# ilirlikalla/Smith-Waterman-FPGA-module

Hardware: AMD Instinct MI355X
Metric: GCUPS (higher is better)
Workload: dtype f16

## Files before the change

### smith-waterman-fpga-module_amd/csrc/swbank_bank.h

```cpp
#ifndef SWBANK_BANK_H
#define SWBANK_BANK_H

#include <dlfcn.h>
#include <hip/hip_runtime.h>
#include <rccl/rccl.h>

#include <algorithm>
#include <cmath>
#include <cstdarg>
#include <cstdio>
#include <cstdlib>
#include <cstring>
#include <atomic>
#include <condition_variable>
#include <functional>
#include <memory>
#include <mutex>
#include <numeric>
#include <thread>
#include <chrono>
#include <vector>
#if defined(__SSE2__)
#include <emmintrin.h>
#endif
// ... 219 lines not shown
      if (stop_.load()) return;
      (*job_)(i);
      pending_.fetch_sub(1, std::memory_order_acq_rel);
    }
  }
  unsigned n_;
  std::vector<std::thread> th_;
  std::mutex m_;
  std::condition_variable cv_;
  const std::function<void(unsigned)>* job_ = nullptr;
  std::atomic<unsigned> pending_{0};
  std::atomic<uint64_t> gen_{0};
  std::atomic<bool> stop_{false};
};

class Launcher {
 public:
  explicit Launcher(int device) : th_([this, device] { loop(device); }) {}
  ~Launcher() {
    {
      std::lock_guard<std::mutex> g(m_);
      stop_ = true;
    }
    cv_.notify_one();
    th_.join();
  }
  void post(std::function<sw_status()> f) {
    {
      std::lock_guard<std::mutex> g(m_);
      q_.push_back(std::move(f));
      ++posted_;
    }
    cv_.notify_one();
  }
  sw_status wait(size_t k) {
    while (done_.load(std::memory_order_acquire) < k) {
#if defined(__SSE2__)
      _mm_pause();
#endif
    }
    return st_.load(std::memory_order_acquire);
  }
  sw_status wait_all() { return wait(posted_); }
  void reset() {
    wait_all();
    posted_ = 0;
    done_.store(0);
    st_.store(SW_OK);
  }

 private:
  void loop(int device) {
    (void)hipSetDevice(device);
    for (;;) {
      std::function<sw_status()> f;
      {
        std::unique_lock<std::mutex> l(m_);
        cv_.wait(l, [&] { return stop_ || !q_.empty(); });
        if (q_.empty()) return;
        f = std::move(q_.front());
        q_.erase(q_.begin());
      }
      if (st_.load(std::memory_order_relaxed) == SW_OK) {
        const sw_status s = f();
        if (s != SW_OK) st_.store(s, std::memory_order_release);
      }
      done_.fetch_add(1, std::memory_order_acq_rel);
    }
  }
  std::mutex m_;
  std::condition_variable cv_;
  std::vector<std::function<sw_status()>> q_;
  bool stop_ = false;
  size_t posted_ = 0;
  std::atomic<size_t> done_{0};
  std::atomic<sw_status> st_{SW_OK};
  std::thread th_;
};

struct sw_bank {
  sw_config cfg{};
  int device = 0;
  int cus = 0;
  hipStream_t stream = nullptr;
  char err[512] = {0};

  bool have_pen = false;
  int alpha = SW_DNA_ALPHA;
  std::vector<int8_t> matrix;
  int32_t gap_open = 0, gap_extend = 0;

  bool have_query = false;
  uint64_t qid = 0;
  std::vector<uint8_t> query;
  std::vector<std::vector<uint8_t>> qset;
  bool mq_ready = false;
  DevBuf<uint32_t> mqtab, mqtab16;
  size_t mq_words = 0;
  DevBuf<uint32_t> mqpair;
  size_t mq_pair_words = 0;
  int mq_pair_segs = 0, mq_pair_rows = 0;
  uint32_t mq_pS1 = 0, mq_pS2 = 0;

  bool dirty = true;
  int R = 32, RB = 4, W = 1, col0 = 0, prof = 0;
  uint32_t S = 0, O = 0, E = 0, nv = 0, PS = 0, pad = 4;
  int32_t smax = 0;
  DevBuf<uint32_t> qtab;
  bool f16 = false;
  uint32_t nv16 = 0, PS16 = 0;
  int32_t f16_neg = 0;
  DevBuf<uint32_t> qtab16;
  DevBuf<uint32_t> qpair;
  uint32_t pair_bytes = 0, pS1 = 0, pS2 = 0;
  DevBuf<uint32_t> fb_idx, fb_cnt;
  bool i32_ready = false;
  uint32_t i32_strips = 0;
  DevBuf<uint2> i32prof, i32scr;
  DevBuf<unsigned long long> best_key;
  struct Seg { int W; size_t off, off16; };
  std::vector<Seg> segs;
  DevBuf<uint2> edge[2];
  int wK = 0;
  int wsegs = 1;
  size_t wseg_words = 0, wseg_words16 = 0;
  uint32_t wPS = 0;
  DevBuf<uint32_t> wtab;
  DevBuf<uint32_t> wtab16;
  uint32_t wPS16 = 0;
  int sK[3] = {0, 0, 0};
  size_t sseg_words[3] = {0, 0, 0}, sseg_words16[3] = {0, 0, 0};
  uint32_t sPS[3] = {0, 0, 0}, sPS16[3] = {0, 0, 0};
  DevBuf<uint32_t> stab[3], stab16[3];
  DevBuf<uint2> sring;
  DevBuf<uint32_t> tprog;

  static constexpr int NSLOT = 3, NDSLOT = 6;
  hipStream_t copy_stream = nullptr;
  hipEvent_t h2d_done[NSLOT] = {}, kern_done[NDSLOT] = {};
  PinBuf hslot[NSLOT], hscores;
  std::vector<std::vector<uint32_t>> mlist;
  std::vector<std::vector<uint8_t>> mstage;
  std::vector<std::vector<uint32_t>> mbad;
  std::vector<hipEvent_t> out_ev;
  hipStream_t out_stream = nullptr;
  hipStream_t stream2 = nullptr;
  hipEvent_t ev_s2 = nullptr;
  double host_pack_ms = 0;
  int feed_dslots = NSLOT;
  DevBuf<uint8_t> dslot[NDSLOT];
  DevBuf<uint32_t> sortscr[NDSLOT];
  DevBuf<uint8_t> sbuf;
  UcBuf sflag;
  DevBuf<SwkStreamChunk> sdrec;
  DevBuf<uint32_t> sctr;
  hipStream_t kstream = nullptr;
  PinBuf srec, shflag{hipHostMallocCoherent};
  PinBuf shscores{hipHostMallocCoherent};
  std::vector<hipEvent_t> sev;
  std::unique_ptr<HostPool> pool;
  std::unique_ptr<Launcher> launcher;

  DevBuf<uint8_t> res;
  DevBuf<uint64_t> offs;
  DevBuf<uint32_t> lens;
  DevBuf<int32_t> scores;
  DevBuf<uint8_t> gres;
  DevBuf<uint64_t> goffs;
  DevBuf<uint32_t> glens;

  char last_kernel[160] = {0};

  int best_kind = 0;
  uint64_t best_id = 0, best_index = 0;
  int32_t best_score = 0;
  DevBuf<uint64_t> best_dev;
  hipEvent_t best_ev = nullptr;

  std::vector<sw_bank*> kids;
  std::unique_ptr<HostPool> dpool;
  std::vector<void*> comms;
  bool rccl_gather = false;
  unsigned pool_threads = 0;
  DevBuf<int32_t> grecv;
  PinBuf hrecv;
  DevBuf<uint32_t> bal_state, bal_flag;
  DevBuf<uint32_t> wbal_state, wbal_flag;
  uint32_t wbal_gen = 0;
  DevBuf<uint32_t> bal_plan;
  size_t bal_key[3] = {0, 0, 0};
  uint32_t bal_gen = 0;
  bool peer_ready = false;
  hipEvent_t ev_join = nullptr;
  std::vector<hipEvent_t> deal_ev;
  bool best_root = false;
  DevBuf<uint32_t> dperm, dsort;
  bool is_multi() const { return !kids.empty(); }
  bool gotoh() const { return cfg.gap_model == SW_GAP_GOTOH; }

  hipEvent_t ev_ready = nullptr, ev_used = nullptr;
  PinBuf stage;

  sw_counters ctr{};

  PinBuf faultw{hipHostMallocCoherent};
  bool host_call = false;
  bool no_handoff = false;

  bool timing = false;
  struct Ev { hipEvent_t a, b, c; };
  std::vector<Ev> events;
};

struct DevGuard {
  int prev = -1;
  DevGuard() {
    if (hipGetDevice(&prev) != hipSuccess) prev = -1;
  }
  explicit DevGuard(const sw_bank* b) : DevGuard() {
    if (b && b->device >= 0) (void)hipSetDevice(b->device);
  }
  ~DevGuard() {
    if (prev >= 0) (void)hipSetDevice(prev);
  }
  DevGuard(const DevGuard&) = delete;
  DevGuard& operator=(const DevGuard&) = delete;
};

inline uint16_t f16_score_bits(int v) {
  return __builtin_bit_cast(uint16_t, (_Float16)((float)v * (1.0f / 2048.0f)));
}


sw_status fail(sw_bank* b, sw_status st, const char* fmt, ...);

#define HIPOK(bank, expr)                                                                 \
  do {                                                                                    \
    hipError_t e_ = (expr);                                                               \
    if (e_ != hipSuccess)                                                                 \
      return fail((bank), SW_ERR_HIP, "%s: %s (%s:%d)", #expr, hipGetErrorString(e_),    \
                  __FILE__, __LINE__);                                                    \
  } while (0)

struct Rccl {
  bool ok = false;
  char err[160] = {0};
  decltype(&ncclCommInitAll) commInitAll = nullptr;
  decltype(&ncclCommDestroy) commDestroy = nullptr;
  decltype(&ncclGather) gather = nullptr;
  decltype(&ncclGetErrorString) errorString = nullptr;
  decltype(&ncclCommAbort) commAbort = nullptr;
  decltype(&ncclCommGetAsyncError) asyncError = nullptr;
  decltype(&ncclGroupStart) groupStart = nullptr;
  decltype(&ncclGroupEnd) groupEnd = nullptr;
};
const Rccl& rccl();

template <class F>
sw_status each_kid(sw_bank* b, F&& f) {
  for (sw_bank* k : b->kids) {
    const sw_status st = f(k);
    if (st != SW_OK) return fail(b, st, "device %d: %s", k->device, k->err);
  }
  return SW_OK;
}

unsigned host_threads();

template <class F>
void parallel_for(HostPool& pool, size_t n, F&& f) {
  const unsigned T = pool.size();
  if (T <= 1 || n < 2048) {
    f((size_t)0, n);
    return;
  }
  const size_t step = (n + T - 1) / T;
  pool.run([&](unsigned p) {
    const size_t lo = std::min(n, p * step), hi = std::min(n, lo + step);
    if (lo < hi) f(lo, hi);
  });
}

inline size_t align16(size_t x) { return (x + 15) & ~(size_t)15; }
inline uint32_t record_len(const uint8_t* rec) {
  uint16_t l;
  std::memcpy(&l, rec + 4, 2);
  return l;
}

void copy_kernel_name(sw_bank* b, const char* gather);
uint32_t* fault_word(sw_bank* b);
sw_status take_fault(sw_bank* b, int which);
sw_status prepare(sw_bank* b);
sw_status prepare_multi(sw_bank* b);
sw_status prepare_i32(sw_bank* b);
void u16_gotoh_rows(const sw_bank* b, bool f16, int& R, int& W);
bool wave_preferred(const sw_bank* b, size_t n, uint32_t max_len, bool use_f16);
sw_status launch(sw_bank* b, const uint8_t* d_res, const uint64_t* d_offs,
                 const uint32_t* d_lens, size_t n, uint32_t max_len, int32_t* d_scores,
                 hipStream_t st, uint32_t packed = SWK_PACK_BYTES,
                 const uint32_t* perm = nullptr, const uint32_t* perm_n = nullptr,
                 bool dsort = false, bool wait_prev = true, uint32_t* sort_out = nullptr,
                 uint32_t* sort_scr = nullptr, uint32_t ulen = 0, uint32_t ustride = 0,
                 uint32_t min_len = 0);
bool chunk_perm(HostPool& pool, const uint32_t* len, size_t n, uint32_t* perm);
bool scratch_free(const sw_bank* b, uint32_t max_len);
struct MixedOrder {
  std::vector<uint32_t> pos;
  uint32_t hi = 0, shift = 0, nbin = 0;
};
bool mixed_pack(sw_bank* b, const uint8_t* residues, size_t nres, const uint64_t* offsets,
                const uint32_t* lens, size_t c0, size_t cnt, size_t step,
// ... 25 lines not shown
```

### smith-waterman-fpga-module_amd/csrc/swbank_bank.hip

```cpp
#include "swbank_bank.h"

sw_status fail(sw_bank* b, sw_status st, const char* fmt, ...) {
  if (b) {
    va_list ap;
    va_start(ap, fmt);
    vsnprintf(b->err, sizeof(b->err), fmt, ap);
    va_end(ap);
  }
  return st;
}

extern "C" int32_t sw_device_count(void) {
  int n = 0;
  if (hipGetDeviceCount(&n) != hipSuccess) return 0;
  return n;
}

static sw_status check_device(int dev) {
  int ndev = 0;
  if (hipGetDeviceCount(&ndev) != hipSuccess || ndev <= 0) return SW_ERR_NO_DEVICE;
  if (dev < 0 || dev >= ndev) return SW_ERR_NO_DEVICE;
  hipDeviceProp_t prop;
  if (hipGetDeviceProperties(&prop, dev) != hipSuccess) return SW_ERR_NO_DEVICE;
  if (std::strncmp(prop.gcnArchName, "gfx950", 6) != 0) return SW_ERR_NO_DEVICE;
// ... 37 lines not shown
      }
      k->pool_threads = std::max(2u, host_threads() / (unsigned)cfg.n_devices);
      b->kids.push_back(k);
    }
    b->dpool.reset(new (std::nothrow) HostPool((unsigned)cfg.n_devices));
    b->pool.reset(new (std::nothrow) HostPool(host_threads()));
    if (!b->dpool || !b->pool) {
      sw_bank_destroy(b);
      return SW_ERR_NOMEM;
    }
    const char* gm = std::getenv("SWBANK_GATHER");
    const bool force_copy = gm && std::strcmp(gm, "copy") == 0;
    const bool force_rccl = gm && std::strcmp(gm, "rccl") == 0;
    bool distinct = true;
    for (int i = 0; i < cfg.n_devices; ++i)
      for (int j = 0; j < i; ++j) distinct = distinct && cfg.devices[i] != cfg.devices[j];
    if (!force_copy && (distinct || force_rccl)) {
      const Rccl& r = rccl();
      ncclResult_t nr = ncclSuccess;
      if (r.ok) {
        std::vector<ncclComm_t> comms((size_t)cfg.n_devices);
        nr = r.commInitAll(comms.data(), cfg.n_devices, cfg.devices);
        if (nr == ncclSuccess) b->comms.assign(comms.begin(), comms.end());
      }
      b->rccl_gather = !b->comms.empty();
      if (b->comms.empty() && force_rccl) {
        sw_bank_destroy(b);
        return SW_ERR_UNSUPPORTED;
      }
      if (b->comms.empty())
        snprintf(b->err, sizeof(b->err), "RCCL unavailable (%s), gathering with device copies",
                 r.ok ? r.errorString(nr) : r.err);
    }
    (void)hipSetDevice(b->device);
    *out = b;
    return SW_OK;
  }

  int dev = cfg.device;
  if (dev < 0 && hipGetDevice(&dev) != hipSuccess) return SW_ERR_NO_DEVICE;
  const sw_status dst = check_device(dev);
  if (dst != SW_OK) return dst;

  sw_bank* b = new (std::nothrow) sw_bank();
  if (!b) return SW_ERR_NOMEM;
  b->cfg = cfg;
  b->device = dev;
  if (hipSetDevice(dev) != hipSuccess ||
      hipStreamCreateWithFlags(&b->stream, hipStreamNonBlocking) != hipSuccess ||
      hipStreamCreateWithFlags(&b->copy_stream, hipStreamNonBlocking) != hipSuccess ||
      hipStreamCreateWithFlags(&b->out_stream, hipStreamNonBlocking) != hipSuccess ||
      hipStreamCreateWithFlags(&b->stream2, hipStreamNonBlocking) != hipSuccess) {
    for (hipStream_t* x : {&b->stream, &b->copy_stream, &b->out_stream, &b->stream2})
      if (*x) (void)hipStreamDestroy(*x);
    delete b;
    return SW_ERR_HIP;
  }
  b->alpha = cfg.alphabet == SW_ALPHABET_DNA ? SW_DNA_ALPHA : SW_PROTEIN_ALPHA;
  if (hipDeviceGetAttribute(&b->cus, hipDeviceAttributeMultiprocessorCount, dev) != hipSuccess)
    b->cus = 0;
  if (cfg.alphabet == SW_ALPHABET_PROTEIN) {
    int8_t m[SW_PROTEIN_ALPHA * SW_PROTEIN_ALPHA];
    sw_fill_matrix(SW_ALPHABET_PROTEIN, 0, 0, m);
    b->matrix.assign(m, m + sizeof(m));
    b->gap_open = -11;
    b->gap_extend = -1;
    b->have_pen = true;
  }
  *out = b;
  return SW_OK;
}

extern "C" void sw_bank_destroy(sw_bank* b) {
  DevGuard dev_guard(b);
  if (!b) return;
  if (b->is_multi() || !b->comms.empty()) {
    const Rccl& r = rccl();
    for (void* c : b->comms) (void)r.commDestroy(static_cast<ncclComm_t>(c));
    (void)hipSetDevice(b->device);
    if (b->ev_used) (void)hipEventSynchronize(b->ev_used);
    if (b->ev_join) (void)hipEventDestroy(b->ev_join);
    if (b->ev_used) (void)hipEventDestroy(b->ev_used);
    for (sw_bank* k : b->kids) sw_bank_destroy(k);
    b->dpool.reset();
    b->pool.reset();
    (void)hipSetDevice(b->device);
    b->grecv.release();
    b->hrecv.release();
    b->res.release();
    b->offs.release();
    b->lens.release();
    b->dperm.release();
    b->dsort.release();
    delete b;
    return;
  }
  (void)hipSetDevice(b->device);
  if (b->stream) (void)hipStreamSynchronize(b->stream);
  uint64_t nl;
  double pm, sm;
  (void)sw_bank_timing(b, &nl, &pm, &sm);
  b->faultw.release();
  b->qtab.release();
  b->qtab16.release();
  b->mqtab.release();
  b->mqtab16.release();
  b->mqpair.release();
  b->qpair.release();
  b->stage.release();
  if (b->ev_ready) (void)hipEventDestroy(b->ev_ready);
  if (b->ev_used) (void)hipEventDestroy(b->ev_used);
  if (b->best_ev) (void)hipEventDestroy(b->best_ev);
  if (b->ev_join) (void)hipEventDestroy(b->ev_join);
  for (hipEvent_t e : b->deal_ev) (void)hipEventDestroy(e);
  b->fb_idx.release();
  b->fb_cnt.release();
  b->best_key.release();
  b->best_dev.release();
  b->i32prof.release();
  b->i32scr.release();
  b->dperm.release();
  b->dsort.release();
  b->bal_state.release();
  b->bal_flag.release();
  b->wbal_state.release();
  b->wbal_flag.release();
  b->bal_plan.release();
  b->wtab.release();
  b->wtab16.release();
  b->tprog.release();
  for (int i = 0; i < 3; ++i) {
    b->stab[i].release();
    b->stab16[i].release();
  }
  b->sring.release();
  b->edge[0].release();
  b->edge[1].release();
  if (b->copy_stream) (void)hipStreamSynchronize(b->copy_stream);
  if (b->out_stream) (void)hipStreamSynchronize(b->out_stream);
  if (b->stream2) (void)hipStreamSynchronize(b->stream2);
  for (hipEvent_t e : b->out_ev) (void)hipEventDestroy(e);
  for (int i = 0; i < sw_bank::NSLOT; ++i) b->hslot[i].release();
  for (int i = 0; i < sw_bank::NDSLOT; ++i) {
    b->dslot[i].release();
    b->sortscr[i].release();
  }
  b->sbuf.release();
  b->sflag.release();
  b->sdrec.release();
  b->sctr.release();
  b->srec.release();
  b->shflag.release();
  b->shscores.release();
  for (hipEvent_t e : b->sev) (void)hipEventDestroy(e);
  for (int i = 0; i < sw_bank::NSLOT; ++i)
    if (b->h2d_done[i]) (void)hipEventDestroy(b->h2d_done[i]);
  for (int i = 0; i < sw_bank::NDSLOT; ++i)
    if (b->kern_done[i]) (void)hipEventDestroy(b->kern_done[i]);
  b->hscores.release();
  b->launcher.reset();
  b->pool.reset();
  if (b->copy_stream) (void)hipStreamDestroy(b->copy_stream);
  if (b->out_stream) (void)hipStreamDestroy(b->out_stream);
  if (b->stream2) (void)hipStreamDestroy(b->stream2);
  if (b->kstream) (void)hipStreamDestroy(b->kstream);
  if (b->ev_s2) (void)hipEventDestroy(b->ev_s2);
  b->res.release();
  b->offs.release();
  b->lens.release();
  b->scores.release();
  b->gres.release();
  b->goffs.release();
  b->glens.release();
  if (b->stream) (void)hipStreamDestroy(b->stream);
  delete b;
}

extern "C" int32_t sw_bank_devices(const sw_bank* b, int32_t* devices, int32_t cap) {
  if (!b) return 0;
  const int32_t n = b->is_multi() ? (int32_t)b->kids.size() : 1;
  for (int32_t i = 0; devices && i < std::min(n, cap); ++i)
    devices[i] = b->is_multi() ? b->kids[(size_t)i]->device : b->device;
  return n;
}

extern "C" const char* sw_last_error(const sw_bank* b) { return b ? b->err : "null bank"; }

extern "C" const char* sw_last_kernel(const sw_bank* b) { return b ? b->last_kernel : ""; }

uint32_t* fault_word(sw_bank* b) {
  if (!b->faultw.p) {
    if (b->faultw.reserve(64) != hipSuccess) return nullptr;
    std::memset(b->faultw.p, 0, b->faultw.cap);
  }
  return reinterpret_cast<uint32_t*>(b->faultw.p);
}

sw_status take_fault(sw_bank* b, int which) {
  if (b->is_multi()) {
    sw_status st = SW_OK;
    for (sw_bank* k : b->kids) {
      const sw_status ks = take_fault(k, which);
      if (ks != SW_OK && st == SW_OK) st = fail(b, ks, "device %d: %s", k->device, k->err);
    }
    return st;
  }
  if (!b->faultw.p) return SW_OK;
  volatile uint32_t* w = reinterpret_cast<volatile uint32_t*>(b->faultw.p) + which * SWK_FAULT_WORDS;
  uint32_t f = 0;
  for (int i = 0; i < SWK_FAULT_WORDS; ++i) {
    f |= w[i];
    w[i] = 0;
  }
  if (f == 0) return SW_OK;
  if (f & SWK_FAULT_BAL) ++b->ctr.balanced_timeouts;
  if (f & SWK_FAULT_TAIL) ++b->ctr.tail_timeouts;
  if (f & SWK_FAULT_WBAL) ++b->ctr.wave_balanced_timeouts;
  char kinds[96] = "";
  const char* names[3] = {"balanced ranges", "protein tail", "wave balanced ranges"};
  for (int i = 0; i < 3; ++i)
    if (f & (1u << i)) {
      if (kinds[0]) strncat(kinds, ", ", sizeof(kinds) - strlen(kinds) - 1);
      strncat(kinds, names[i], sizeof(kinds) - strlen(kinds) - 1);
    }
  return fail(b, SW_ERR_TIMEOUT,
              "a cross-workgroup hand-off wait ran out (%s) in a %s call: its scores are invalid",
              kinds, which ? "host-buffer" : "device");
}

extern "C" sw_status sw_bank_sync(sw_bank* b) {
  DevGuard dev_guard(b);
  if (!b) return SW_ERR_ARG;
  if (b->is_multi()) {
    for (sw_bank* k : b->kids) {
      const sw_status st = sw_bank_sync(k);
      if (st != SW_OK) {
        (void)take_fault(b, 0);
        return fail(b, st, "device %d: %s", k->device, k->err);
      }
    }
    if (b->ev_used) {
      int cur = -1;
      HIPOK(b, hipGetDevice(&cur));
      hipError_t e = hipSetDevice(b->device);
      if (e == hipSuccess) e = hipEventSynchronize(b->ev_used);
      (void)hipSetDevice(cur);
      HIPOK(b, e);
    }
    return SW_OK;
  }
  int cur = -1;
  HIPOK(b, hipGetDevice(&cur));
  hipError_t e = hipSetDevice(b->device);
  if (e == hipSuccess && b->ev_used) e = hipEventSynchronize(b->ev_used);
  if (e == hipSuccess) e = hipStreamSynchronize(b->stream);
  (void)hipSetDevice(cur);
  HIPOK(b, e);
  return take_fault(b, 0);
}

static void sum_counters(sw_counters& c, const sw_bank* b) {
  c.stream_calls += b->ctr.stream_calls;
  c.stream_reruns += b->ctr.stream_reruns;
  c.stream_declined += b->ctr.stream_declined;
  c.chunked_calls += b->ctr.chunked_calls;
  c.device_sorts += b->ctr.device_sorts;
  c.gather_timeouts += b->ctr.gather_timeouts;
  c.mixed_chunks += b->ctr.mixed_chunks;
  c.mixed_runs += b->ctr.mixed_runs;
  c.balanced_calls += b->ctr.balanced_calls;
  c.balanced_timeouts += b->ctr.balanced_timeouts;
  c.tail_timeouts += b->ctr.tail_timeouts;
  c.handoff_reruns += b->ctr.handoff_reruns;
  c.wave_balanced_timeouts += b->ctr.wave_balanced_timeouts;
  c.h2d_bytes += __atomic_load_n(&b->ctr.h2d_bytes, __ATOMIC_RELAXED);
}

extern "C" sw_status sw_bank_counters_ex(const sw_bank* b, sw_counters* out, size_t out_size) {
  if (!b || !out) return SW_ERR_ARG;
  if (out_size != 64 && out_size != 80 && out_size != 96 && out_size != sizeof(sw_counters))
    return SW_ERR_ARG;
  sw_counters c{};
  sum_counters(c, b);
  for (const sw_bank* k : b->kids) sum_counters(c, k);
  std::memcpy(out, &c, out_size);
  return SW_OK;
}

extern "C" sw_status sw_bank_counters(const sw_bank* b, sw_counters* out) {
  return sw_bank_counters_ex(b, out, 64);
}

void copy_kernel_name(sw_bank* b, const char* gather) {
  snprintf(b->last_kernel, sizeof(b->last_kernel), "multi[%zu] gather=%s: %s", b->kids.size(),
           gather, b->kids[0]->last_kernel);
}

static sw_status set_matrix_impl(sw_bank* b, const int8_t* m, int alpha, int32_t go,
                                 int32_t ge) {
  if (go > 0 || ge > 0 || go < -32767 || ge < -32767)
    return fail(b, SW_ERR_ARG, "gap penalties must be <= 0 (got open %d, extend %d)", go, ge);
  b->matrix.assign(m, m + (size_t)alpha * alpha);
  b->alpha = alpha;
  b->gap_open = go;
  b->gap_extend = ge;
  b->have_pen = true;
  b->dirty = true;
// ... 578 lines not shown
```

### smith-waterman-fpga-module_amd/csrc/swbank_kcommon.h

```cpp
#ifndef SWBANK_KCOMMON_H
#define SWBANK_KCOMMON_H
#include <hip/hip_runtime.h>
#include <stdint.h>

#include <algorithm>
#include <cstdlib>
#include <mutex>
#include <type_traits>
#include <vector>

#include "swbank_internal.h"

#ifndef SWK_TAIL_TOP
#define SWK_TAIL_TOP 1
#endif
#ifndef SWK_PRIO_ROT
#define SWK_PRIO_ROT 1
#endif
#ifndef SWK_PRIO_SHIFT
#define SWK_PRIO_SHIFT 18
#endif

#ifndef SWK_PRIO_END
#define SWK_PRIO_END 3
// ... 467 lines not shown
                                              uint32_t ulen, uint32_t ustride) {
  Lane2 t;
  size_t a = (size_t)tile * SWB_TILE + lane, b = a + 64;
  const bool va = a < n, vb = b < n;
  const size_t p0 = (size_t)tile * SWB_TILE;
  if (p0 >= n) {
    t.llo = t.lhi = 0u;
    t.plo = t.phi = packed == SWK_PACK_RECORDS || ustride ? res + (packed ? 6 : 0)
                                                          : reinterpret_cast<const uint8_t*>(lens);
    return t;
  }
  if (!va) a = p0;
  if (!vb) b = p0;
  if (idx) {
    a = idx[a];
    b = idx[b];
  }
  if (packed == SWK_PACK_RECORDS) {
    t.llo = va ? record_len(res + a * SWB_RECORD) : 0u;
    t.lhi = vb ? record_len(res + b * SWB_RECORD) : 0u;
    t.plo = res + a * SWB_RECORD + 6;
    t.phi = res + b * SWB_RECORD + 6;
    return t;
  }
  if (ustride) {
    t.llo = va ? ulen : 0u;
    t.lhi = vb ? ulen : 0u;
    t.plo = res + a * ustride;
    t.phi = res + b * ustride;
    return t;
  }
  const uint32_t la = lens[a], lb = lens[b];
  t.llo = va ? la : 0u;
  t.lhi = vb ? lb : 0u;
  if constexpr (MIX) {
    if (packed == SWK_PACK_MIXED) {
      const uint32_t* o32 = reinterpret_cast<const uint32_t*>(offs);
      t.plo = la ? mixed_ptr(res, o32[a]) : reinterpret_cast<const uint8_t*>(lens);
      t.phi = lb ? mixed_ptr(res, o32[b]) : reinterpret_cast<const uint8_t*>(lens);
      return t;
    }
  }
  t.plo = la ? res + offs[a] : reinterpret_cast<const uint8_t*>(lens);
  t.phi = lb ? res + offs[b] : reinterpret_cast<const uint8_t*>(lens);
  return t;
}

template <int C = 8>
__device__ __forceinline__ void tile_chunks(const Lane2& t, size_t tlo, size_t thi, size_t n,
                                            int& nch, int& nfull, int& ncl) {
  uint32_t Lmax = max(t.llo, t.lhi);
  uint32_t Lmin = min(tlo < n ? t.llo : ~0u, thi < n ? t.lhi : ~0u);
#pragma unroll
  for (int off = 32; off >= 1; off >>= 1) {
    Lmax = max(Lmax, (uint32_t)__shfl_xor((int)Lmax, off));
    Lmin = min(Lmin, (uint32_t)__shfl_xor((int)Lmin, off));
  }
  const int lx = (int)__builtin_amdgcn_readfirstlane(Lmax);
  nch = max(1, (lx + C - 1) / C);
  ncl = lx == 0 ? C : lx - C * (nch - 1);
  const uint32_t lm = __builtin_amdgcn_readfirstlane(Lmin);
  nfull = lm == ~0u ? 0 : (int)(lm / C);
}

struct ScoreArgs {
  const uint8_t* res;
  const uint64_t* offs;
  const uint32_t* lens;
  size_t n;
  const uint32_t* qtab;
  uint32_t nv;
  uint32_t S, O, E;
  uint32_t PS;
  uint32_t pad;
  int32_t* scores;
  const uint2* edge_in;
  uint2* edge_out;
  uint32_t ecols;
  uint32_t accum;
  uint32_t packed;
  const uint32_t* idx;
  const uint32_t* nidx;
  uint32_t idx_base;
  const uint32_t* ident;
  uint32_t pS1, pS2;
  uint32_t f16_noe, f16_ne, f16_no;
  const uint32_t* fb_qtab;
  uint32_t fb_nv, fb_PS;
  int32_t fb_thresh;
  uint32_t split_blocks;
  uint32_t split_P;
  uint32_t main_pairs;
  const uint32_t* split_qtab;
  const uint32_t* split_fb_qtab;
  uint32_t split_words, split_fb_words, split_PS, split_fb_PS;
  uint2* split_ring;
  uint32_t ulen, ustride;
  uint32_t nq, qwords;
  size_t sstride;
  const SwkStreamChunk* sc;
  const uint32_t* hflag;
  uint32_t* dflag;
  uint32_t* tctr;
  uint32_t nsc;
  uint32_t* bal_flag;
  uint32_t* bal_state;
  const uint4* bal_plan;
  uint32_t bal_gen;
  uint32_t* tail_prog;
  uint32_t tail_pairs, tail_cols;
  uint32_t* fault;
  uint32_t poll_limit, stall;
  uint32_t wbal_blocks, wbal_grid;
  const uint32_t* sidx;
};
static_assert(sizeof(ScoreArgs) == 376, "ScoreArgs layout (kernel argument block) changed");

__device__ __forceinline__ void report_fault(uint32_t* fault, uint32_t bit) {
  if (fault) __hip_atomic_store(fault + __builtin_ctz(bit), bit, __ATOMIC_RELAXED,
                                __HIP_MEMORY_SCOPE_SYSTEM);
}

typedef __attribute__((address_space(3))) void* lds_void_ptr;
typedef __attribute__((address_space(1))) void* glob_void_ptr;

template <int C = 8>
__device__ __forceinline__ void dma_edge_chunk(const uint2* src, uint2* dst, int lane) {
#pragma unroll
  for (int q = 0; q < C / 2; ++q)
    __builtin_amdgcn_global_load_lds((glob_void_ptr)(src + q * 128 + lane * 2),
                                     (lds_void_ptr)(dst + q * 128), 16, 0, 0);
}

template <int C = 8>
__device__ __forceinline__ int tile_nch(const uint8_t* res, const uint32_t* lens, size_t n,
                                        int tile, int lane, uint32_t packed, const uint32_t* idx,
                                        uint32_t ulen, uint32_t ustride) {
  const size_t a = (size_t)tile * SWB_TILE + lane, b = a + 64;
  auto len = [&](size_t k) -> uint32_t {
    if (k >= n) return 0u;
    if (ustride) return ulen;
    if (idx) k = idx[k];
    return packed == SWK_PACK_RECORDS ? record_len(res + k * SWB_RECORD) : lens[k];
  };
  uint32_t L = max(len(a), len(b));
#pragma unroll
  for (int off = 32; off >= 1; off >>= 1) L = max(L, (uint32_t)__shfl_xor((int)L, off));
  return max(1, (int)((__builtin_amdgcn_readfirstlane(L) + C - 1) / C));
}

#ifndef SWK_STREAM_POLL
#define SWK_STREAM_POLL 64
#endif
#ifndef SWK_STREAM_POLL_ALL
#define SWK_STREAM_POLL_ALL 0
#endif
__device__ __forceinline__ uint32_t stream_mode(const uint32_t* hflag, uint32_t* dflag, int c,
                                                int nsc, int lane) {
  for (int it = 0; it < (1 << 20); ++it) {
    uint32_t v = __builtin_amdgcn_readfirstlane(
        __hip_atomic_load(dflag + c, __ATOMIC_ACQUIRE, __HIP_MEMORY_SCOPE_AGENT));
    if (v) {
      __builtin_amdgcn_fence(__ATOMIC_ACQUIRE, "");
      return v;
    }
    if ((SWK_STREAM_POLL_ALL || threadIdx.x < 64) &&
        (it == 0 || ((it + (int)blockIdx.x) % SWK_STREAM_POLL) == 0)) {
      v = __builtin_amdgcn_readfirstlane(
          __hip_atomic_load(hflag + c, __ATOMIC_ACQUIRE, __HIP_MEMORY_SCOPE_SYSTEM));
      if (v) {
        if (lane == 0) __hip_atomic_store(dflag + c, v, __ATOMIC_RELEASE, __HIP_MEMORY_SCOPE_AGENT);
        return v;
      }
    }
    __builtin_amdgcn_s_sleep(16);
  }
  if (lane == 0) {
    __hip_atomic_store(dflag + c, SWK_STREAM_ABORT, __ATOMIC_RELAXED, __HIP_MEMORY_SCOPE_AGENT);
    __hip_atomic_store(const_cast<uint32_t*>(hflag) + nsc + c, SWK_STREAM_ABORT,
                       __ATOMIC_RELAXED, __HIP_MEMORY_SCOPE_SYSTEM);
  }
  return SWK_STREAM_ABORT;
}


inline int cached_occupancy(const void* fn, int threads, size_t lds, int dev, int* cus) {
  struct Entry { const void* fn; int threads; size_t lds; int dev, occ, cus; };
  static std::mutex m;
  static std::vector<Entry> cache;
  std::lock_guard<std::mutex> g(m);
  for (const Entry& e : cache)
    if (e.fn == fn && e.threads == threads && e.lds == lds && e.dev == dev) {
      *cus = e.cus;
      return e.occ;
    }
  int occ = 0, c = 0;
  if (hipDeviceGetAttribute(&c, hipDeviceAttributeMultiprocessorCount, dev) != hipSuccess ||
      hipOccupancyMaxActiveBlocksPerMultiprocessor(&occ, fn, threads, lds) != hipSuccess)
    return 0;
  cache.push_back({fn, threads, lds, dev, occ, c});
  *cus = c;
  return occ;
}

inline unsigned persistent_grid(const void* fn, size_t ntiles, int threads, size_t lds) {
  int dev = 0, cus = 0;
  if (hipGetDevice(&dev) != hipSuccess) return (unsigned)ntiles;
  const int occ = cached_occupancy(fn, threads, lds, dev, &cus);
  if (cus <= 0 || occ <= 0) return (unsigned)ntiles;
  const size_t slots = (size_t)cus * occ;
  const size_t rounds = (ntiles + slots - 1) / slots;
  return (unsigned)((ntiles + rounds - 1) / rounds);
}

}
#endif
```

### smith-waterman-fpga-module_amd/csrc/swbank_stream.hip

```cpp
#include "swbank_bank.h"

sw_status stream_feed(sw_bank* b, const uint8_t* residues, size_t nres,
                      const uint64_t* offsets, size_t n, uint32_t L, int32_t* out, bool& used,
                      const uint8_t* recs, const uint32_t* rlens) {
  used = false;
  if (recs && (L == 0 || L > SWB_RECORD_MAX)) return SW_OK;
  const int mode_env = env_int("SWBANK_STREAM", 1);
  if (mode_env == 0 || !out || b->alpha != SW_DNA_ALPHA || b->prof || b->col0 || b->RB != 4 ||
      env_int("SWBANK_PACK2", 1) == 0 || env_int("SWBANK_UNIFORM", 1) == 0 ||
      !scratch_free(b, L) || n > 0x7FFFFFFFull)
    return SW_OK;
  if (rlens && env_int("SWBANK_MIXED", 1) == 0) return SW_OK;
  const char* kforce = std::getenv("SWBANK_KERNEL");
  if (kforce && std::strcmp(kforce, "wave") == 0) return SW_OK;
  const size_t T = (n + SWB_TILE - 1) / SWB_TILE;
  if (mode_env != 2 && T < 8 * (size_t)std::max(b->cus, 1)) return SW_OK;
  const uint64_t smax = (uint64_t)std::max(0, b->smax);
  const bool use_f16 = b->f16 && b->f16_neg >= -2048 && env_int("SWBANK_F16", 1) != 0 &&
                       std::min<uint64_t>(b->query.size(), L) * smax + smax <= 2048u;
  const bool pair = use_f16 && b->pair_bytes != 0 && env_int("SWBANK_PAIR", 1) != 0;
  if (!(b->R == 16 || b->R == 32)) return SW_OK;
  int sR = b->R, sW = b->segs[0].W;
  u16_gotoh_rows(b, use_f16, sR, sW);

  std::vector<size_t> tile0;
  const size_t cap = std::max<size_t>(1, T / 8);
  for (size_t t = 0, sz = std::max<size_t>(1, T / 64); t < T; t += sz, sz = std::min(cap, 2 * sz))
    tile0.push_back(t);
  const size_t nsc = tile0.size();
  tile0.push_back(T);
  const size_t nib = (L + 1) / 2;
  const size_t PT0 = b->pool ? b->pool->size() : 1;
  std::vector<size_t> roff(nsc + 1, 0);
  size_t slot_bytes = 0, zbytes = 0;
  for (size_t i = 0; i < nsc; ++i) {
    const size_t cnt = std::min(n, tile0[i + 1] * SWB_TILE) - tile0[i] * SWB_TILE;
    const size_t head = rlens ? align16(cnt * 12) : 0;
    const size_t body = rlens ? cnt * ((L + 3) / 4) + cnt * (size_t)L / 32 + cnt * nib + 32 * PT0
                              : cnt * nib;
    if (rlens && head + body + 64 >= ((size_t)1 << 29)) return SW_OK;
    roff[i + 1] = roff[i] + (head + body + 64 + 255) / 256 * 256;
    slot_bytes = std::max(slot_bytes, roff[i + 1] - roff[i]);
    zbytes = std::max(zbytes, head + 64);
  }
  if (!rlens) zbytes = 0;
  const size_t cap_bytes = (size_t)std::max(1, env_int("SWBANK_STREAM_MB", 4096)) << 20;
  if (roff[nsc] + zbytes + n * 4 > cap_bytes) {
    ++b->ctr.stream_declined;
    return SW_OK;
  }
  HIPOK(b, hipSetDevice(b->device));
  if (!b->kstream) {
    if (b->cus <= 0) return SW_OK;
    std::vector<uint32_t> mask(((size_t)b->cus + 31) / 32, 0xFFFFFFFFu);
    if (hipExtStreamCreateWithCUMask(&b->kstream, (uint32_t)mask.size(), mask.data()) !=
        hipSuccess) {
      b->kstream = nullptr;
      (void)hipGetLastError();
      return SW_OK;
    }
  }
  hipStream_t ks = b->kstream;
  {
    bool ok = b->sbuf.reserve(roff[nsc] + zbytes) == hipSuccess &&
              b->sflag.reserve(nsc * 4) == hipSuccess &&
              b->sdrec.reserve(nsc) == hipSuccess && b->sctr.reserve(1) == hipSuccess &&
              b->srec.reserve(nsc * sizeof(SwkStreamChunk)) == hipSuccess &&
              b->shflag.reserve(nsc * 8) == hipSuccess &&
              b->shscores.reserve(n * 4) == hipSuccess;
    for (int i = 0; ok && i < std::min<int>(sw_bank::NSLOT, (int)nsc); ++i)
      ok = b->hslot[i].reserve(slot_bytes) == hipSuccess;
    while (ok && b->sev.size() < nsc) {
      hipEvent_t e;
      ok = hipEventCreateWithFlags(&e, hipEventDisableTiming | hipEventBlockingSync) == hipSuccess;
      if (ok) b->sev.push_back(e);
    }
    if (!ok) {
      (void)hipGetLastError();
      b->sbuf.release();
      b->shscores.release();
      ++b->ctr.stream_declined;
      return SW_OK;
    }
  }
  used = true;
  SwkStreamChunk* rec = reinterpret_cast<SwkStreamChunk*>(b->srec.p);
  uint32_t* hflag = reinterpret_cast<uint32_t*>(b->shflag.p);
  for (size_t i = 0; i < nsc; ++i) {
    rec[i] = SwkStreamChunk{(unsigned)tile0[i], (unsigned)roff[i], (unsigned)(roff[i] >> 32),
                            (unsigned)(roff[nsc] / 256)};
    __atomic_store_n(&hflag[i], 0u, __ATOMIC_RELAXED);
    __atomic_store_n(&hflag[nsc + i], 0u, __ATOMIC_RELAXED);
  }
  std::atomic_thread_fence(std::memory_order_seq_cst);

  sw_bank::Ev ev{};
  const auto start_kernel = [&]() -> sw_status {
    HIPOK(b, hipStreamWaitEvent(ks, b->ev_ready, 0));
    HIPOK(b, hipStreamWaitEvent(ks, b->ev_used, 0));
    HIPOK(b, hipMemcpyAsync(b->sdrec.p, rec, nsc * sizeof(SwkStreamChunk), hipMemcpyHostToDevice,
                            ks));
    HIPOK(b, hipMemsetAsync(b->sflag.p, 0, nsc * 4, ks));
    HIPOK(b, hipMemsetAsync(b->sctr.p, 0, 4, ks));
    if (zbytes) HIPOK(b, hipMemsetAsync(b->sbuf.p + roff[nsc], 0, zbytes, ks));
    if (b->timing) {
      HIPOK(b, hipEventCreate(&ev.a));
      HIPOK(b, hipEventCreate(&ev.c));
      HIPOK(b, hipEventRecord(ev.a, ks));
      ev.b = ev.a;
    }
    HIPOK(b, swk_launch_stream(sR, b->gotoh() ? 1 : 0, use_f16 ? 1 : 0, pair ? 1 : 0, b->sbuf.p,
                               n, rlens ? 0u : L, b->sdrec.p, hflag,
                               reinterpret_cast<uint32_t*>(b->sflag.p),
                               (uint32_t)nsc, b->sctr.p,
                               pair ? b->qpair.p : use_f16 ? b->qtab16.p : b->qtab.p,
                               use_f16 ? b->nv16 : b->nv, b->S, b->O, b->E,
                               pair ? b->pair_bytes : 0, b->pad, sW,
                               reinterpret_cast<int32_t*>(b->shscores.p),
                               b->pS1, b->pS2, ks));
    HIPOK(b, hipEventRecord(b->ev_used, ks));
    if (b->timing) {
      HIPOK(b, hipEventRecord(ev.c, ks));
      b->events.push_back(ev);
    }
    snprintf(b->last_kernel, sizeof(b->last_kernel), "tile %s%s R=%d W=%d segs=1 streamed=%zu",
             use_f16 ? "f16" : "u16", pair ? " pair" : "", sR, sW, nsc);
    trace_mark("kernel");
    return SW_OK;
  };

  std::vector<uint32_t> mode(nsc, 0);
  size_t issued = 0;
  bool stop = false;
  std::mutex pm;
  std::condition_variable pcv;
  const int hold_ms = env_int("SWBANK_STREAM_HOLD_MS", 0);
  std::vector<std::chrono::steady_clock::time_point> pub_t(nsc);
  size_t published = 0;
  hipError_t pub_err = hipSuccess;
  std::thread publisher([&] {
    for (size_t i = 0; i < nsc; ++i) {
      {
        std::unique_lock<std::mutex> lk(pm);
        pcv.wait(lk, [&] { return issued > i || stop; });
        if (issued <= i) return;
      }
      const hipError_t e = hipEventSynchronize(b->sev[i]);
      if (e != hipSuccess) {
        pub_err = e;
        for (size_t j = i; j < nsc; ++j) __atomic_store_n(&hflag[j], SWK_STREAM_ABORT, __ATOMIC_RELEASE);
        return;
      }
      if (i == 1 && hold_ms > 0) std::this_thread::sleep_for(std::chrono::milliseconds(hold_ms));
      __atomic_store_n(&hflag[i], mode[i], __ATOMIC_RELEASE);
      pub_t[i] = std::chrono::steady_clock::now();
      published = i + 1;
    }
  });

  HostPool& pool = *b->pool;
  const unsigned PT = pool.size();
  const bool avx2 = env_int("SWBANK_AVX2", 1) != 0;
  const swpack::PackFn pack2fn = swpack::packer(2, avx2), pack4fn = swpack::packer(4, avx2);
  const size_t steps32 = (L + 31u) / 32u;
  bool nib_mode = false;
  std::atomic<size_t> oob{SIZE_MAX};
  std::vector<uint64_t> rbase(PT), rspan(PT);
  std::vector<size_t> psz(PT + 1, 0), p4(PT + 1, 0);
  const bool runs_ok = env_int("SWBANK_MIXED_RUNS", 1) != 0;
  MixedOrder mo;
  if (rlens) {
    mo.hi = L;
    while ((L >> mo.shift) >= 1024u) ++mo.shift;
    mo.nbin = (L >> mo.shift) + 1;
    mo.pos.assign((size_t)PT * mo.nbin, 0u);
  }
  std::atomic<uint32_t> wide{0};
  sw_status err = SW_OK;
  bool started = false;
  bool nonuniform = false;
  for (size_t i = 0; i < nsc && err == SW_OK; ++i) {
    const int s = (int)(i % sw_bank::NSLOT);
    if (i >= (size_t)sw_bank::NSLOT) {
      const hipError_t e = hipEventSynchronize(b->h2d_done[s]);
      if (e != hipSuccess) {
        fail(b, SW_ERR_HIP, "hipEventSynchronize: %s", hipGetErrorString(e));
        err = SW_ERR_HIP;
        break;
      }
    }
    const size_t c0 = tile0[i] * SWB_TILE, c1 = std::min(n, tile0[i + 1] * SWB_TILE);
    const size_t cnt = c1 - c0, step = (cnt + PT - 1) / PT;
    uint8_t* codes = b->hslot[s].p;
    trace_mark("gather<");
    const auto t0 = std::chrono::steady_clock::now();
    uint32_t md = 0;
    size_t sb = 0, bytes = 0;
    if (rlens) {
      const size_t ca = align16(cnt * 12);
      uint32_t* so32 = reinterpret_cast<uint32_t*>(codes);
      uint32_t* sl32 = so32 + cnt;
      uint32_t* sp = sl32 + cnt;
      std::fill(mo.pos.begin(), mo.pos.end(), 0u);
      pool.run([&](unsigned p) {
        const size_t lo = std::min(cnt, p * step), hi = std::min(cnt, (p + 1) * step);
        size_t a1 = 0, a2 = 0, a4 = 0;
        bool mono = runs_ok;
        uint64_t first = UINT64_MAX, last = 0;
        uint32_t* h = mo.pos.data() + (size_t)p * mo.nbin;
        for (size_t j = lo; j < hi; ++j) {
          const size_t k = c0 + j;
          const uint32_t l = rlens[k];
          if (offsets[k] > nres || l > nres - offsets[k]) {
            size_t cur = oob.load();
            while (k < cur && !oob.compare_exchange_weak(cur, k)) {
            }
            return;
          }
          a1 += l;
          a2 += (l + 3) / 4;
          a4 += (l + 1) / 2;
          ++h[(mo.hi - std::min(l, mo.hi)) >> mo.shift];
          if (l) {
            mono &= first == UINT64_MAX || offsets[k] >= last;
            if (first == UINT64_MAX) first = offsets[k];
            last = offsets[k] + l;
          }
        }
        const uint64_t span = first == UINT64_MAX ? 0 : last - first;
        const bool run = mono && first != UINT64_MAX && span <= a1 + a1 / 8 + 64 &&
                         span < (1ull << 30);
        rbase[p] = run ? first : UINT64_MAX;
        rspan[p] = run ? span : 0;
        psz[p + 1] = run ? (span + 3) / 4 : a2;
        p4[p + 1] = a4;
      });
      if (oob.load() == SIZE_MAX) {
        for (unsigned p = 0; p < PT; ++p) {
          psz[p + 1] += psz[p];
          p4[p + 1] += p4[p];
        }
        uint32_t at = 0;
        for (uint32_t bin = 0; bin < mo.nbin; ++bin)
          for (unsigned p = 0; p < PT; ++p) {
            uint32_t& x = mo.pos[(size_t)p * mo.nbin + bin];
            const uint32_t c = x;
            x = at;
            at += c;
          }
        size_t end = 0;
        if (mixed_pack(b, residues, nres, offsets, rlens, c0, cnt, step, rbase, rspan, psz, p4,
                       so32, sl32, codes + ca, sp, &mo, end)) {
          md = SWK_PACK_MIXED;
          bytes = ca + end;
          ++b->ctr.mixed_chunks;
        }
      }
      if (oob.load() == SIZE_MAX && md == 0) {
        for (size_t j = 0; j < cnt && err == SW_OK; ++j)
          for (uint32_t x = 0; x < rlens[c0 + j]; ++x)
            if (residues[offsets[c0 + j] + x] >= (uint8_t)SW_DNA_ALPHA) {
              fail(b, SW_ERR_ARG, "target %zu code %u outside alphabet", c0 + j,
                   (unsigned)residues[offsets[c0 + j] + x]);
              err = SW_ERR_ARG;
              break;
            }
        if (err == SW_OK) err = fail(b, SW_ERR_ARG, "code outside alphabet");
        break;
      }
    } else if (recs) {
      sb = (L + 3) / 4;
      std::atomic<bool> other{false};
      const size_t step = (cnt + PT - 1) / PT;
      pool.run([&](unsigned p) {
        const size_t lo = std::min(cnt, p * step), hi = std::min(cnt, (p + 1) * step);
        for (size_t j = lo; j < hi; ++j) {
          const uint8_t* r = recs + (c0 + j) * SWB_RECORD;
          uint16_t l;
          std::memcpy(&l, r + 4, 2);
          if (l != L) {
            other = true;
            return;
          }
          std::memcpy(codes + j * sb, r + 6, sb);
        }
      });
      if (other.load()) {
        nonuniform = true;
        break;
      }
      md = SWK_PACK_STREAM;
    }
    for (int pass = nib_mode ? 1 : 0; !recs && !rlens && pass < 2 && md == 0; ++pass) {
      sb = pass == 0 ? (L + 3) / 4 : nib;
      const size_t stepb = pass == 0 ? 8 : 16;
      const swpack::PackFn fn = pass == 0 ? pack2fn : pack4fn;
      wide = 0;
      const bool runs = (pass == 0 ? L % 4 == 0 : L % 2 == 0) &&
                        env_int("SWBANK_STREAM_RUNS", 1) != 0;
      pool.run([&](unsigned p) {
        const size_t lo = std::min(cnt, p * step), hi = std::min(cnt, (p + 1) * step);
        uint32_t acc = 0;
        if (runs && hi > lo && (hi - lo) * (size_t)L < 0x80000000ull) {
          const uint64_t o0 = offsets[c0 + lo];
          const size_t total = (hi - lo) * (size_t)L;
          bool back = o0 <= nres && total <= nres - o0;
          for (size_t j = lo + 1; back && j < hi; ++j)
            back = offsets[c0 + j] == o0 + (j - lo) * (uint64_t)L;
          if (back) {
            acc = fn(residues + o0, (uint32_t)total, codes + lo * sb, total % 32 == 0);
            if (pass == 0 ? acc > 3u : acc >= (uint32_t)SW_DNA_ALPHA) wide = 1;
            return;
          }
        }
        for (size_t j = lo; j < hi; ++j) {
          const size_t k = c0 + j;
          if (offsets[k] > nres || L > nres - offsets[k]) {
            size_t cur = oob.load();
            while (k < cur && !oob.compare_exchange_weak(cur, k)) {
            }
            return;
          }
          const bool w = offsets[k] + steps32 * 32 <= nres && j * sb + steps32 * stepb <= hi * sb;
          const uint32_t v = fn(residues + offsets[k], L, codes + j * sb, w);
          acc = pass == 0 ? (acc | v) : std::max(acc, v);
        }
        if (pass == 0 ? acc > 3u : acc >= (uint32_t)SW_DNA_ALPHA) wide = 1;
      });
      if (oob.load() != SIZE_MAX) break;
      if (wide.load() == 0) md = pass == 0 ? SWK_PACK_STREAM : SWK_PACK_NIBBLE;
      else if (pass == 0) nib_mode = true;
    }
    if (b->timing)
      b->host_pack_ms +=
          std::chrono::duration<double, std::milli>(std::chrono::steady_clock::now() - t0).count();
    trace_mark("gather>");
    if (oob.load() != SIZE_MAX) {
      const size_t k = oob.load();
      fail(b, SW_ERR_ARG, "target %zu [%llu, +%u) outside the %zu residues", k,
           (unsigned long long)offsets[k], L, nres);
      err = SW_ERR_ARG;
      break;
    }
    if (md == 0) {
      for (size_t j = 0; j < cnt && err == SW_OK; ++j)
        for (uint32_t x = 0; x < L; ++x)
          if (residues[offsets[c0 + j] + x] >= (uint8_t)SW_DNA_ALPHA) {
            fail(b, SW_ERR_ARG, "target %zu code %u outside alphabet", c0 + j,
                 (unsigned)residues[offsets[c0 + j] + x]);
            err = SW_ERR_ARG;
            break;
          }
      if (err == SW_OK) err = fail(b, SW_ERR_ARG, "code outside alphabet");
      break;
    }
    if (!rlens) bytes = cnt * sb;
    std::memset(codes + bytes, 0, 16);
    const hipError_t e1 = hipMemcpyAsync(b->sbuf.p + roff[i], codes, bytes + 16,
                                         hipMemcpyHostToDevice, b->copy_stream);
    __atomic_fetch_add(&b->ctr.h2d_bytes, (uint64_t)(bytes + 16), __ATOMIC_RELAXED);
    const hipError_t e2 = e1 != hipSuccess ? e1 : hipEventRecord(b->h2d_done[s], b->copy_stream);
    const hipError_t e3 = e2 != hipSuccess ? e2 : hipEventRecord(b->sev[i], b->copy_stream);
    if (e3 != hipSuccess) {
      fail(b, SW_ERR_HIP, "streamed chunk copy: %s", hipGetErrorString(e3));
      err = SW_ERR_HIP;
      break;
    }
    mode[i] = md;
    {
      std::lock_guard<std::mutex> lk(pm);
      issued = i + 1;
    }
    pcv.notify_one();
    trace_mark("launched");
    if (i == 0 && (err = start_kernel()) != SW_OK) break;
    started = i == 0 || started;
  }
  {
    std::lock_guard<std::mutex> lk(pm);
    stop = true;
  }
  pcv.notify_one();
  publisher.join();
  if (g_trace)
    for (size_t i = 0; i < published; ++i) g_trace->mark_at("published", pub_t[i]);
  for (size_t i = issued; i < nsc; ++i)
    __atomic_store_n(&hflag[i], SWK_STREAM_ABORT, __ATOMIC_RELEASE);
  if (!started) {
    (void)hipStreamSynchronize(b->copy_stream);
    if (nonuniform) used = false;
    return err;
  }
  const hipError_t se = hipStreamSynchronize(ks);
  if (err != SW_OK) return err;
  if (pub_err != hipSuccess)
    return fail(b, SW_ERR_HIP, "streamed chunk copy: %s", hipGetErrorString(pub_err));
  if (nonuniform) {
    used = false;
    return SW_OK;
  }
  if (se != hipSuccess) return fail(b, SW_ERR_HIP, "streamed batch: %s", hipGetErrorString(se));
  trace_mark("landed");
  for (size_t i = 0; i < nsc; ++i)
    if (__atomic_load_n(&hflag[nsc + i], __ATOMIC_ACQUIRE) == SWK_STREAM_ABORT) {
      used = false;
      ++b->ctr.stream_reruns;
      return SW_OK;
    }
  ++b->ctr.stream_calls;
  const int32_t* hs = reinterpret_cast<const int32_t*>(b->shscores.p);
  std::vector<size_t> pbest(PT, SIZE_MAX);
  const size_t ostep = (n + PT - 1) / PT;
  pool.run([&](unsigned p) {
    const size_t lo = std::min(n, p * ostep), hi = std::min(n, (p + 1) * ostep);
    size_t bi = lo;
    for (size_t k = lo; k < hi; ++k) {
      const int32_t v = hs[k];
      out[k] = v;
      if (v > hs[bi]) bi = k;
    }
    if (lo < hi) pbest[p] = bi;
  });
  size_t best = 0;
  for (size_t x : pbest)
    if (x != SIZE_MAX && hs[x] > hs[best]) best = x;
  b->best_index = best;
  b->best_id = best;
  b->best_score = hs[best];
  b->best_kind = 1;
  trace_mark("done");
  return SW_OK;
}
```

Baseline: 12590.

## Publish streamed chunk readiness via in-stream flag copies instead of publisher thread

Removes the host publisher thread that waited on a per-chunk event and then wrote a host-visible flag. The copy stream now writes each chunk's mode word straight into the device flag buffer right after the chunk data copy, so the kernel sees readiness through its device-scope poll. Host-flag polling in the kernel becomes rarer, skipping the first-iteration check. Device flags are cleared by an H2D copy ordered with an event, replacing the memset on the kernel stream. This cuts host thread wakeups and event-sync latency, but relies on copies on the same stream landing in order and being visible to a kernel that is already running.

```diff
diff --git a/smith-waterman-fpga-module_amd/csrc/swbank_bank.h b/smith-waterman-fpga-module_amd/csrc/swbank_bank.h
--- a/smith-waterman-fpga-module_amd/csrc/swbank_bank.h
+++ b/smith-waterman-fpga-module_amd/csrc/swbank_bank.h
@@ -395,12 +395,12 @@
   DevBuf<uint32_t> sortscr[NDSLOT];
   DevBuf<uint8_t> sbuf;
   UcBuf sflag;
+  hipEvent_t sflag_clear = nullptr;
   DevBuf<SwkStreamChunk> sdrec;
   DevBuf<uint32_t> sctr;
   hipStream_t kstream = nullptr;
   PinBuf srec, shflag{hipHostMallocCoherent};
   PinBuf shscores{hipHostMallocCoherent};
-  std::vector<hipEvent_t> sev;
   std::unique_ptr<HostPool> pool;
   std::unique_ptr<Launcher> launcher;
 
diff --git a/smith-waterman-fpga-module_amd/csrc/swbank_bank.hip b/smith-waterman-fpga-module_amd/csrc/swbank_bank.hip
--- a/smith-waterman-fpga-module_amd/csrc/swbank_bank.hip
+++ b/smith-waterman-fpga-module_amd/csrc/swbank_bank.hip
@@ -213,7 +213,7 @@
   b->srec.release();
   b->shflag.release();
   b->shscores.release();
-  for (hipEvent_t e : b->sev) (void)hipEventDestroy(e);
+  if (b->sflag_clear) (void)hipEventDestroy(b->sflag_clear);
   for (int i = 0; i < sw_bank::NSLOT; ++i)
     if (b->h2d_done[i]) (void)hipEventDestroy(b->h2d_done[i]);
   for (int i = 0; i < sw_bank::NDSLOT; ++i)
diff --git a/smith-waterman-fpga-module_amd/csrc/swbank_kcommon.h b/smith-waterman-fpga-module_amd/csrc/swbank_kcommon.h
--- a/smith-waterman-fpga-module_amd/csrc/swbank_kcommon.h
+++ b/smith-waterman-fpga-module_amd/csrc/swbank_kcommon.h
@@ -643,9 +643,6 @@
 #ifndef SWK_STREAM_POLL
 #define SWK_STREAM_POLL 64
 #endif
-#ifndef SWK_STREAM_POLL_ALL
-#define SWK_STREAM_POLL_ALL 0
-#endif
 __device__ __forceinline__ uint32_t stream_mode(const uint32_t* hflag, uint32_t* dflag, int c,
                                                 int nsc, int lane) {
   for (int it = 0; it < (1 << 20); ++it) {
@@ -655,8 +652,7 @@
       __builtin_amdgcn_fence(__ATOMIC_ACQUIRE, "");
       return v;
     }
-    if ((SWK_STREAM_POLL_ALL || threadIdx.x < 64) &&
-        (it == 0 || ((it + (int)blockIdx.x) % SWK_STREAM_POLL) == 0)) {
+    if (threadIdx.x < 64 && ((it + (int)blockIdx.x) % SWK_STREAM_POLL) == SWK_STREAM_POLL - 1) {
       v = __builtin_amdgcn_readfirstlane(
           __hip_atomic_load(hflag + c, __ATOMIC_ACQUIRE, __HIP_MEMORY_SCOPE_SYSTEM));
       if (v) {
diff --git a/smith-waterman-fpga-module_amd/csrc/swbank_stream.hip b/smith-waterman-fpga-module_amd/csrc/swbank_stream.hip
--- a/smith-waterman-fpga-module_amd/csrc/swbank_stream.hip
+++ b/smith-waterman-fpga-module_amd/csrc/swbank_stream.hip
@@ -66,15 +66,12 @@
               b->sflag.reserve(nsc * 4) == hipSuccess &&
               b->sdrec.reserve(nsc) == hipSuccess && b->sctr.reserve(1) == hipSuccess &&
               b->srec.reserve(nsc * sizeof(SwkStreamChunk)) == hipSuccess &&
-              b->shflag.reserve(nsc * 8) == hipSuccess &&
+              b->shflag.reserve(nsc * 16) == hipSuccess &&
               b->shscores.reserve(n * 4) == hipSuccess;
     for (int i = 0; ok && i < std::min<int>(sw_bank::NSLOT, (int)nsc); ++i)
       ok = b->hslot[i].reserve(slot_bytes) == hipSuccess;
-    while (ok && b->sev.size() < nsc) {
-      hipEvent_t e;
-      ok = hipEventCreateWithFlags(&e, hipEventDisableTiming | hipEventBlockingSync) == hipSuccess;
-      if (ok) b->sev.push_back(e);
-    }
+    if (ok && !b->sflag_clear)
+      ok = hipEventCreateWithFlags(&b->sflag_clear, hipEventDisableTiming) == hipSuccess;
     if (!ok) {
       (void)hipGetLastError();
       b->sbuf.release();
@@ -91,16 +88,21 @@
                             (unsigned)(roff[nsc] / 256)};
     __atomic_store_n(&hflag[i], 0u, __ATOMIC_RELAXED);
     __atomic_store_n(&hflag[nsc + i], 0u, __ATOMIC_RELAXED);
-  }
+    hflag[3 * nsc + i] = 0u;
+  }
+  uint32_t* const mode = hflag + 2 * nsc;
   std::atomic_thread_fence(std::memory_order_seq_cst);
+  HIPOK(b, hipMemcpyAsync(b->sflag.p, hflag + 3 * nsc, nsc * 4, hipMemcpyHostToDevice,
+                          b->copy_stream));
+  HIPOK(b, hipEventRecord(b->sflag_clear, b->copy_stream));
 
   sw_bank::Ev ev{};
   const auto start_kernel = [&]() -> sw_status {
     HIPOK(b, hipStreamWaitEvent(ks, b->ev_ready, 0));
     HIPOK(b, hipStreamWaitEvent(ks, b->ev_used, 0));
+    HIPOK(b, hipStreamWaitEvent(ks, b->sflag_clear, 0));
     HIPOK(b, hipMemcpyAsync(b->sdrec.p, rec, nsc * sizeof(SwkStreamChunk), hipMemcpyHostToDevice,
                             ks));
-    HIPOK(b, hipMemsetAsync(b->sflag.p, 0, nsc * 4, ks));
     HIPOK(b, hipMemsetAsync(b->sctr.p, 0, 4, ks));
     if (zbytes) HIPOK(b, hipMemsetAsync(b->sbuf.p + roff[nsc], 0, zbytes, ks));
     if (b->timing) {
@@ -129,34 +131,8 @@
     return SW_OK;
   };
 
-  std::vector<uint32_t> mode(nsc, 0);
   size_t issued = 0;
-  bool stop = false;
-  std::mutex pm;
-  std::condition_variable pcv;
   const int hold_ms = env_int("SWBANK_STREAM_HOLD_MS", 0);
-  std::vector<std::chrono::steady_clock::time_point> pub_t(nsc);
-  size_t published = 0;
-  hipError_t pub_err = hipSuccess;
-  std::thread publisher([&] {
-    for (size_t i = 0; i < nsc; ++i) {
-      {
-        std::unique_lock<std::mutex> lk(pm);
-        pcv.wait(lk, [&] { return issued > i || stop; });
-        if (issued <= i) return;
-      }
-      const hipError_t e = hipEventSynchronize(b->sev[i]);
-      if (e != hipSuccess) {
-        pub_err = e;
-        for (size_t j = i; j < nsc; ++j) __atomic_store_n(&hflag[j], SWK_STREAM_ABORT, __ATOMIC_RELEASE);
-        return;
-      }
-      if (i == 1 && hold_ms > 0) std::this_thread::sleep_for(std::chrono::milliseconds(hold_ms));
-      __atomic_store_n(&hflag[i], mode[i], __ATOMIC_RELEASE);
-      pub_t[i] = std::chrono::steady_clock::now();
-      published = i + 1;
-    }
-  });
 
   HostPool& pool = *b->pool;
   const unsigned PT = pool.size();
@@ -360,30 +336,23 @@
                                          hipMemcpyHostToDevice, b->copy_stream);
     __atomic_fetch_add(&b->ctr.h2d_bytes, (uint64_t)(bytes + 16), __ATOMIC_RELAXED);
     const hipError_t e2 = e1 != hipSuccess ? e1 : hipEventRecord(b->h2d_done[s], b->copy_stream);
-    const hipError_t e3 = e2 != hipSuccess ? e2 : hipEventRecord(b->sev[i], b->copy_stream);
+    if (e2 == hipSuccess && i == 1 && hold_ms > 0)
+      std::this_thread::sleep_for(std::chrono::milliseconds(hold_ms));
+    mode[i] = md;
+    const hipError_t e3 =
+        e2 != hipSuccess ? e2
+                         : hipMemcpyAsync(b->sflag.p + i * 4, &mode[i], 4, hipMemcpyHostToDevice,
+                                          b->copy_stream);
     if (e3 != hipSuccess) {
       fail(b, SW_ERR_HIP, "streamed chunk copy: %s", hipGetErrorString(e3));
       err = SW_ERR_HIP;
       break;
     }
-    mode[i] = md;
-    {
-      std::lock_guard<std::mutex> lk(pm);
-      issued = i + 1;
-    }
-    pcv.notify_one();
-    trace_mark("launched");
+    issued = i + 1;
+    trace_mark("published");
     if (i == 0 && (err = start_kernel()) != SW_OK) break;
     started = i == 0 || started;
   }
-  {
-    std::lock_guard<std::mutex> lk(pm);
-    stop = true;
-  }
-  pcv.notify_one();
-  publisher.join();
-  if (g_trace)
-    for (size_t i = 0; i < published; ++i) g_trace->mark_at("published", pub_t[i]);
   for (size_t i = issued; i < nsc; ++i)
     __atomic_store_n(&hflag[i], SWK_STREAM_ABORT, __ATOMIC_RELEASE);
   if (!started) {
@@ -392,9 +361,9 @@
     return err;
   }
   const hipError_t se = hipStreamSynchronize(ks);
+  if (err != SW_OK || nonuniform)
+    (void)hipStreamSynchronize(b->copy_stream);
   if (err != SW_OK) return err;
-  if (pub_err != hipSuccess)
-    return fail(b, SW_ERR_HIP, "streamed chunk copy: %s", hipGetErrorString(pub_err));
   if (nonuniform) {
     used = false;
     return SW_OK;
@@ -405,6 +374,7 @@
     if (__atomic_load_n(&hflag[nsc + i], __ATOMIC_ACQUIRE) == SWK_STREAM_ABORT) {
       used = false;
       ++b->ctr.stream_reruns;
+      (void)hipStreamSynchronize(b->copy_stream);
       return SW_OK;
     }
   ++b->ctr.stream_calls;
```

Result: no change. 12550 (-0.3%).
